# qianlim/CAPE

Hardware: AMD Instinct MI355X
Metric: meshes/sec fwd+bwd, CAPE-affineconv nz64 @ batch 16, 1/2/4/8 MI355X (higher is better)
Workload: dtype f32

## Files before the change

cape_amd/csrc/gconv.hip:

```cpp
#include "common.h"
#include "gconv_shared.h"
#include "gemm_plain.h"
#include "gemm_split.h"
#include "gemm_h2.h"
#include "narrow.h"
#include <stdlib.h>
#include <algorithm>
#include <vector>

namespace {

constexpr int KC_DEFAULT = 32;

template <int ROWS, int LDA, int KC, typename AT = float>
__device__ __forceinline__ void stage_rows(float *sA, const SrcDev &S, int n, int r0, int Mo,
                                            int c0, int tid) {
    constexpr int QPR = KC / 4;
    constexpr int RP = 256 / QPR;
    const int q = tid % QPR;
    const int rl0 = tid / QPR;
    const int c = c0 + 4 * q;
    const AT *x0 = reinterpret_cast<const AT *>(S.x) + (long long)n * S.xs;
    const AT *xb = x0 + c;
    const int nvalid = S.C - c;
// ... 489 lines not shown
    return CAPE_OK;
}

inline int fill_h2(GconvParams &p, const cape_h2_t *h2, bool dual, int out_deinterleave) {
    p.wsi = p.wsi2 = nullptr;
    p.rm_out = nullptr;
    p.rm_out_w = 0;
    if (!h2) return CAPE_OK;
    if (h2->rowmax_out) {
        if (out_deinterleave > 1 || h2->rowmax_out_w < (p.F + 31) / 32 || (h2->rowmax_out_w & 3)) return CAPE_EINVAL;
        p.rm_out = h2->rowmax_out;
        p.rm_out_w = h2->rowmax_out_w;
    }
    if (!h2->src) return CAPE_OK;
    p.wsi = h2->wscale_inv;
    p.wsi2 = dual ? h2->w2scale_inv : nullptr;
    for (int i = 0; i < p.nsrc; ++i) {
        const cape_h2_src_t &h = h2->src[i];
        SrcDev &d = p.s[i];
        d.wh = h.w_hi; d.wl = h.w_lo; d.wp = h.w_pitch;
        d.wh2 = d.w2 ? h.w2_hi : nullptr; d.wl2 = d.w2 ? h.w2_lo : nullptr; d.wp2 = h.w2_pitch;
        d.rm = h.rowmax; d.rmw = h.rowmax_w;
    }
    return CAPE_OK;
}

struct DwPlan {
    int ct, ft, ctiles[CAPE_MAX_SRC], ftiles, ntiles, rsplit, rows_per_split, ngroups, samples_per_group;
    int vstart[CAPE_MAX_SRC + 1];
    long long slab;
};

constexpr int DW_SLOTS_SERIAL = 512, DW_SLOTS_PIPELINED = 256;
inline void plan_dw_splits(int N, int Mo, DwPlan &pl, int slots = DW_SLOTS_SERIAL) {
    int S = slots / pl.ntiles;
    if (S < 1) S = 1;
    int ngroups = 1;
    for (int d = 1; d <= N && d <= S; ++d)
        if (N % d == 0) ngroups = d;
    const int maxr = (Mo + 127) / 128;
    int rsplit = S / ngroups;
    if (rsplit > maxr) rsplit = maxr;
    if (rsplit < 1) rsplit = 1;
    int rows = (Mo + rsplit - 1) / rsplit;
    rows = ((rows + 31) / 32) * 32;
    pl.rows_per_split = rows;
    pl.rsplit = (Mo + rows - 1) / rows;
    pl.samples_per_group = N / ngroups;
    pl.ngroups = ngroups;
}

inline void plan_dw(const cape_src_t *srcs, int nsrc, int N, int Mo, int F, DwPlan &pl) {
    int maxC = 0;
    for (int i = 0; i < nsrc; ++i) maxC = srcs[i].C > maxC ? srcs[i].C : maxC;
    pl.ct = (maxC <= 64) ? 64 : 128;
    pl.ft = (F <= 64) ? 64 : 128;
    pl.ftiles = (F + pl.ft - 1) / pl.ft;
    pl.ntiles = 0;
    pl.slab = 0;
    for (int i = 0; i < nsrc; ++i) {
        pl.ctiles[i] = (srcs[i].C + pl.ct - 1) / pl.ct;
        pl.ntiles += pl.ctiles[i] * pl.ftiles;
        pl.slab += (long long)srcs[i].C * F;
    }
    plan_dw_splits(N, Mo, pl);
}

inline void plan_dw_plain(const cape_src_t *srcs, int nsrc, int N, int Mo, int F, bool pack, DwPlan &pl) {
    int sumC = 0, maxC = 0;
    pl.slab = 0;
    for (int i = 0; i < nsrc; ++i) {
        sumC += srcs[i].C;
        maxC = srcs[i].C > maxC ? srcs[i].C : maxC;
        pl.slab += (long long)srcs[i].C * F;
    }
    const int span = pack ? sumC : maxC;
    const int n128 = (span + 127) / 128, n64 = (span + 63) / 64;
    pl.ft = (F <= 32) ? 32 : (F <= 64) ? 64 : 128;
    pl.ct = (pl.ft == 32 || n64 == 2 * n128) ? 128 : 64;
    pl.ftiles = (F + pl.ft - 1) / pl.ft;
    int v = 0;
    for (int i = 0; i < nsrc; ++i) {
        if (!pack) v = (v + pl.ct - 1) / pl.ct * pl.ct;
        pl.vstart[i] = v;
        v += srcs[i].C;
    }
    pl.vstart[nsrc] = v;
    pl.ntiles = ((v + pl.ct - 1) / pl.ct) * pl.ftiles;
    plan_dw_splits(N, Mo, pl);
}

inline bool dw_srcs_plain(const cape_src_t *srcs, int nsrc, int es = 4) {
    for (int i = 0; i < nsrc; ++i)
        if ((((srcs[i].C + 3) & ~3) > srcs[i].ldx) || (srcs[i].ldx & 3) || (srcs[i].x_sample_stride & 3) ||
            (reinterpret_cast<uintptr_t>(srcs[i].x) & (4 * es - 1)))
            return false;
    return true;
}


inline bool dw_dz_vec(const float *dz, int64_t dz_sample_stride, int32_t lddz, const float *dz2, int es = 4) {
    return ((lddz & 3) == 0) && ((dz_sample_stride & 3) == 0) && ((reinterpret_cast<uintptr_t>(dz) & (4 * es - 1)) == 0) &&
           (!dz2 || (reinterpret_cast<uintptr_t>(dz2) & (4 * es - 1)) == 0);
}

inline void fill_h2_dw(DwParams &p, const cape_h2_dw_t *h2) {
    p.dzrm = p.dz2rm = nullptr;
    p.dzrmw = p.dz2rmw = 0;
    if (!h2) return;
    for (int i = 0; i < p.nsrc; ++i) { p.s[i].rm = h2->src_rowmax[i]; p.s[i].rmw = h2->src_rowmax_w[i]; }
    p.dzrm = h2->dz_rowmax; p.dzrmw = h2->dz_rowmax_w;
    p.dz2rm = h2->dz2_rowmax; p.dz2rmw = h2->dz2_rowmax_w;
}

inline int choose_dw(const cape_src_t *srcs, int nsrc, const float *dz, int64_t dz_sample_stride, int32_t lddz,
                     const float *dz2, uint32_t dz2_mask, int N, int Mo, int F, DwPlan &pl, bool bf16 = false) {
    static const int dwp_on = getenv("CAPE_DW_PLAIN") ? atoi(getenv("CAPE_DW_PLAIN")) : 1;
    const int es = bf16 ? 2 : 4;
    const bool dzvec = dw_dz_vec(dz, dz_sample_stride, lddz, dz2, es);
    const bool plain = dwp_on && dzvec && (((F + 3) & ~3) <= lddz) && dw_srcs_plain(srcs, nsrc, es);
    if (bf16) {
        bool c4b = true;
        int sumCb = 0;
        for (int i = 0; i < nsrc; ++i) { c4b = c4b && (srcs[i].C & 3) == 0; sumCb += srcs[i].C; }
        if (plain && c4b && (F & 1) == 0) {
            plan_dw(srcs, nsrc, N, Mo, F, pl);
            return 3;
        }
        if (plain && c4b && !(dz2 && dz2_mask) && nsrc > 1 && sumCb <= 128 && F <= 64) {
            plan_dw_plain(srcs, nsrc, N, Mo, F, true, pl);
            return 2;
        }
        plan_dw(srcs, nsrc, N, Mo, F, pl);
        return plain ? 1 : 0;
    }
    int sumC = 0;
    for (int i = 0; i < nsrc; ++i) sumC += srcs[i].C;
    bool c4 = true;
    for (int i = 0; i < nsrc; ++i) c4 = c4 && (srcs[i].C & 3) == 0;
    const bool packed = plain && c4 && !(dz2 && dz2_mask) && nsrc > 1 && sumC <= 128 && F <= 64;
    static const int dws_on = getenv("CAPE_DW_BF16X6") ? atoi(getenv("CAPE_DW_BF16X6")) : CAPE_DW_BF16X6_DEFAULT;
    const bool dw_split = dws_on && plain && !packed && c4 && (F & 1) == 0;
    if (packed) plan_dw_plain(srcs, nsrc, N, Mo, F, true, pl);
    else plan_dw(srcs, nsrc, N, Mo, F, pl);
    return packed ? 2 : dw_split ? 3 : plain ? 1 : 0;
}

struct FwdPlan {
    int family;
    int BM, BN;
    int layout;
};

inline FwdPlan plan_fwd(const GconvParams &p, const cape_src_t *srcs, bool dual, bool bf16 = false) {
    FwdPlan pl;
    static const int gp_on = getenv("CAPE_GEMM_PLAIN") ? atoi(getenv("CAPE_GEMM_PLAIN")) : 1;
    pl.layout = gp_on ? gp_weight_layout(p, dual) : -1;
    if (bf16) {
        bool ok = pl.layout >= 0 && p.F >= 64;
        for (int i = 0; i < p.nsrc && ok; ++i) {
            const long long ws = srcs[i].w_cs > srcs[i].w_rs ? srcs[i].w_cs : srcs[i].w_rs;
            ok = (srcs[i].ldx & 7) == 0 && (srcs[i].x_sample_stride & 7) == 0 && (reinterpret_cast<uintptr_t>(srcs[i].x) & 15) == 0 &&
                 (long long)p.Mo * srcs[i].ldx < (1LL << 31) && (long long)p.F * ws < (1LL << 31) &&
                 srcs[i].C % GS_KC == 0 && srcs[i].C >= GS_KC;
        }
        if (ok) {
            pl.family = 2;
            gs_tile(dual, p.N, p.Mo, p.F, pl.BM, pl.BN);
            return pl;
        }
        pl.layout = -1;
    }
    for (int i = 0; i < p.nsrc && pl.layout >= 0; ++i) {
        const long long ws = srcs[i].w_cs > srcs[i].w_rs ? srcs[i].w_cs : srcs[i].w_rs;
        if ((long long)p.Mo * srcs[i].ldx >= (1LL << 31) || (long long)p.F * ws >= (1LL << 31)) pl.layout = -1;
    }
    if (pl.layout >= 0 && h2_eligible(p, dual)) {
        pl.family = 3;
        pl.layout = 1;
        int ktot = 0;
        for (int i = 0; i < p.nsrc; ++i) ktot += p.s[i].C;
        h2_tile(dual, p.N, p.Mo, p.F, ktot, pl.BM, pl.BN);
        return pl;
    }
    if (pl.layout >= 0) {
        static const int gs_on = getenv("CAPE_GEMM_BF16X6") ? atoi(getenv("CAPE_GEMM_BF16X6")) : CAPE_GEMM_BF16X6_DEFAULT;
        if (gs_on && gs_eligible(p, dual)) {
            pl.family = 2;
            gs_tile(dual, p.N, p.Mo, p.F, pl.BM, pl.BN);
            return pl;
        }
        static const int narrow_on = getenv("CAPE_NARROW") ? atoi(getenv("CAPE_NARROW")) : 1;
        int sumC = 0;
        for (int i = 0; i < p.nsrc; ++i) sumC += p.s[i].C;
        if (narrow_on && !dual && sumC <= NARROW_MAXC && (p.F & 3) == 0 && p.F >= 16 && p.F <= 256 &&
            (long long)p.N * p.Mo < (1LL << 31)) {
            pl.family = 4;
            pl.BM = 256 / narrow_lpr(p.F / 4); pl.BN = p.F;
            return pl;
        }
        pl.family = 1;
        gp_tile(dual, p.F, pl.BM, pl.BN);
        return pl;
    }
    pl.family = 0;
    pl.BN = (p.F <= 32) ? 32 : (p.F <= 64 || dual) ? 64 : 128;
    pl.BM = 128;
    constexpr int bm64_below = 640;
    if (pl.BN == 128 && (long long)p.N * ((p.Mo + 127) / 128) * ((p.F + 127) / 128) < bm64_below) pl.BM = 64;
    return pl;
}

inline int fill_fwd_srcs(GconvParams &p, const cape_src_t *srcs, int nsrc, bool &dual, int es = 4) {
    dual = false;
    for (int i = 0; i < nsrc; ++i) {
        if (!srcs[i].w) return CAPE_EINVAL;
        int rc = fill_src(p.s[i], srcs[i], es);
        if (rc) return rc;
        dual = dual || (srcs[i].w2 != nullptr);
    }
    p.nsrc = nsrc;
    return CAPE_OK;
}

}

namespace {

int gconv_fwd_plan_impl(const cape_src_t *srcs, int32_t nsrc, int32_t N, int32_t Mo, int32_t F, int32_t plan[4], bool bf16,
                        const cape_h2_t *h2 = nullptr) {
    if (!srcs || nsrc < 1 || nsrc > CAPE_MAX_SRC || N < 1 || Mo < 1 || F < 1 || !plan) return CAPE_EINVAL;
    GconvParams p;
    bool dual;
    int rc = fill_fwd_srcs(p, srcs, nsrc, dual, bf16 ? 2 : 4);
    if (rc) return rc;
    p.N = N; p.Mo = Mo; p.F = F;
    rc = fill_h2(p, bf16 ? nullptr : h2, dual, 0);
    if (rc) return rc;
    const FwdPlan pl = plan_fwd(p, srcs, dual, bf16);
    plan[0] = pl.family; plan[1] = pl.BM; plan[2] = pl.BN; plan[3] = pl.family ? pl.layout : 0;
    return CAPE_OK;
}

template <typename AT>
void launch_generic_fwd(const GconvParams &p, const FwdPlan &pl, bool dual, dim3 grid, hipStream_t st) {
    const dim3 block(256);
    if (!dual) {
        if (pl.BN == 32) CAPE_LAUNCH((gconv_fwd_kernel<128, 32, 4, 1, false, KC_DEFAULT, AT>), grid, block, 0, st, p);
        else if (pl.BN == 64) CAPE_LAUNCH((gconv_fwd_kernel<128, 64, 4, 1, false, KC_DEFAULT, AT>), grid, block, 0, st, p);
        else if (pl.BM == 64) CAPE_LAUNCH((gconv_fwd_kernel<64, 128, 2, 2, false, KC_DEFAULT, AT>), grid, block, 0, st, p);
        else CAPE_LAUNCH((gconv_fwd_kernel<128, 128, 2, 2, false, KC_DEFAULT, AT>), grid, block, 0, st, p);
    } else {
        if (pl.BN == 32) CAPE_LAUNCH((gconv_fwd_kernel<128, 32, 4, 1, true, KC_DEFAULT, AT>), grid, block, 0, st, p);
        else CAPE_LAUNCH((gconv_fwd_kernel<128, 64, 4, 1, true, KC_DEFAULT, AT>), grid, block, 0, st, p);
    }
}

int gconv_fwd_impl(const cape_src_t *srcs, int32_t nsrc, float *y, int64_t y_sample_stride,
                   int32_t ldy, int32_t N, int32_t Mo, int32_t F, const float *bias,
                   int32_t bias_mode, int32_t act, uint32_t *mask_out, const cape_rank_t *rank,
                   int32_t out_deinterleave, void *stream, bool bf16, const cape_h2_t *h2 = nullptr) {
    if (!srcs || nsrc < 1 || nsrc > CAPE_MAX_SRC || !y || N < 1 || Mo < 1 || F < 1) return CAPE_EINVAL;
    if (bf16 && h2) return CAPE_EINVAL;
    const int dK = out_deinterleave > 1 ? out_deinterleave : 1;
    const int dstride = dK > 1 ? ((F / dK + 3) & ~3) : 0;
    if (dK > 1 && (F % dK != 0 || mask_out || rank || ldy < dK * dstride)) return CAPE_EINVAL;
    if (dK == 1 && ldy < F) return CAPE_EINVAL;
    if (bias_mode != CAPE_BIAS_NONE && !bias) return CAPE_EINVAL;
    if (act < CAPE_ACT_NONE || act > CAPE_ACT_TANH) return CAPE_EINVAL;
    GconvParams p;
    bool dual;
    int rc = fill_fwd_srcs(p, srcs, nsrc, dual, bf16 ? 2 : 4);
    if (rc) return rc;
    if (mask_out && !dual) return CAPE_EINVAL;
    if (dual && (bias_mode != CAPE_BIAS_NONE || act != CAPE_ACT_NONE)) return CAPE_EINVAL;
    p.y = y; p.ys = y_sample_stride; p.ldy = ldy;
    p.N = N; p.Mo = Mo; p.F = F;
    p.bias = bias; p.bias_mode = bias ? bias_mode : CAPE_BIAS_NONE; p.act = act;
    p.mask = mask_out; p.mask_words = (F + 31) / 32;
    p.rankR = 0; p.rowscale = nullptr; p.coef = nullptr; p.rank_to2 = 0;
    p.deintK = dK; p.deint_stride = dstride;
    if (rank && rank->R > 0) {
        if (rank->R > CAPE_MAX_SRC || !rank->rowscale || !rank->coef) return CAPE_EINVAL;
        if (rank->to_acc2 && !dual) return CAPE_EINVAL;
        p.rankR = rank->R; p.rowscale = rank->rowscale; p.coef = rank->coef; p.rank_to2 = rank->to_acc2;
    }
    rc = fill_h2(p, h2, dual, dK);
    if (rc) return rc;
    FwdPlan pl = plan_fwd(p, srcs, dual, bf16);
    if (pl.family == 4) {
        const bool ok = !p.rankR && !p.mask && dK == 1 && !p.rm_out && (ldy & 3) == 0 && (y_sample_stride & 3) == 0 &&
                        (reinterpret_cast<uintptr_t>(y) & 15) == 0 && (!p.bias || (reinterpret_cast<uintptr_t>(p.bias) & 15) == 0);
        if (ok) {
            const int lpr = narrow_lpr(F / 4), RL = 256 / lpr;
            long long blocks = ((long long)N * Mo + 4 * RL - 1) / (4 * RL);
            if (blocks > 1024) blocks = 1024;
            CAPE_LAUNCH(fwd_narrow_in_kernel, dim3((unsigned)blocks), dim3(256), (size_t)NARROW_MAXC * 4 * lpr * sizeof(float),
                        (hipStream_t)stream, p, lpr);
            CAPE_LAUNCH_CHECK();
            return CAPE_OK;
        }
        pl.family = 1;
        gp_tile(dual, p.F, pl.BM, pl.BN);
    }
    p.row_tiles = (Mo + pl.BM - 1) / pl.BM;
    p.col_tiles = (F + pl.BN - 1) / pl.BN;
    dim3 grid((unsigned)(N * p.row_tiles * p.col_tiles));
    hipStream_t st = (hipStream_t)stream;
    if (pl.family == 3) {
        h2_launch(p, dual, pl.BM, pl.BN, grid, st);
    } else if (pl.family == 2) {
        gs_launch(p, dual, pl.BM, pl.layout, bf16, grid, st);
    } else if (pl.family == 1) {
        gp_launch(p, dual, pl.BM, pl.BN, pl.layout, grid, st);
    } else if (bf16) {
        launch_generic_fwd<cape_bf16>(p, pl, dual, grid, st);
    } else {
        launch_generic_fwd<float>(p, pl, dual, grid, st);
    }
    CAPE_LAUNCH_CHECK();
    return CAPE_OK;
}

}

extern "C" int cape_gconv_fwd_plan(const cape_src_t *srcs, int32_t nsrc, int32_t N, int32_t Mo, int32_t F, int32_t plan[4]) {
    return gconv_fwd_plan_impl(srcs, nsrc, N, Mo, F, plan, false);
}

extern "C" int cape_gconv_fwd_plan_bf16(const cape_src_t *srcs, int32_t nsrc, int32_t N, int32_t Mo, int32_t F, int32_t plan[4]) {
    return gconv_fwd_plan_impl(srcs, nsrc, N, Mo, F, plan, true);
}

extern "C" int cape_gconv_fwd(const cape_src_t *srcs, int32_t nsrc, float *y, int64_t y_sample_stride,
                              int32_t ldy, int32_t N, int32_t Mo, int32_t F, const float *bias,
                              int32_t bias_mode, int32_t act, uint32_t *mask_out, const cape_rank_t *rank,
                              int32_t out_deinterleave, void *stream) {
    return gconv_fwd_impl(srcs, nsrc, y, y_sample_stride, ldy, N, Mo, F, bias, bias_mode, act, mask_out, rank, out_deinterleave,
                          stream, false);
}

extern "C" int cape_gconv_fwd_h2(const cape_src_t *srcs, int32_t nsrc, float *y, int64_t y_sample_stride,
                                 int32_t ldy, int32_t N, int32_t Mo, int32_t F, const float *bias,
                                 int32_t bias_mode, int32_t act, uint32_t *mask_out, const cape_rank_t *rank,
                                 int32_t out_deinterleave, const cape_h2_t *h2, void *stream) {
    return gconv_fwd_impl(srcs, nsrc, y, y_sample_stride, ldy, N, Mo, F, bias, bias_mode, act, mask_out, rank, out_deinterleave,
                          stream, false, h2);
}

extern "C" int cape_gconv_fwd_plan_h2(const cape_src_t *srcs, int32_t nsrc, int32_t N, int32_t Mo, int32_t F, const cape_h2_t *h2,
                                      int32_t plan[4]) {
    return gconv_fwd_plan_impl(srcs, nsrc, N, Mo, F, plan, false, h2);
}

extern "C" int cape_gconv_fwd_bf16(const cape_src_t *srcs, int32_t nsrc, void *y, int64_t y_sample_stride,
                                   int32_t ldy, int32_t N, int32_t Mo, int32_t F, const float *bias,
                                   int32_t bias_mode, int32_t act, uint32_t *mask_out, const cape_rank_t *rank,
                                   int32_t out_deinterleave, void *stream) {
    return gconv_fwd_impl(srcs, nsrc, (float *)y, y_sample_stride, ldy, N, Mo, F, bias, bias_mode, act, mask_out, rank,
                          out_deinterleave, stream, true);
}

extern "C" int64_t cape_gconv_dw_workspace_bytes(const cape_src_t *srcs, int32_t nsrc, int32_t N,
                                                 int32_t Mo, int32_t F) {
    if (!srcs || nsrc < 1 || nsrc > CAPE_MAX_SRC || N < 1 || Mo < 1 || F < 1) return CAPE_EINVAL;
    DwPlan pl;
    plan_dw(srcs, nsrc, N, Mo, F, pl);
    long long need = pl.slab * pl.ngroups * pl.rsplit;
    {
        plan_dw_plain(srcs, nsrc, N, Mo, F, true, pl);
        const long long n2 = pl.slab * pl.ngroups * pl.rsplit;
        need = n2 > need ? n2 : need;
    }
    return (int64_t)need * (int64_t)sizeof(float);
}

namespace {
inline bool dw_takes_h2(const cape_src_t *srcs, int nsrc, const float *dz2, uint32_t dz2_mask, int Mo, int lddz, const cape_h2_dw_t *h2) {
    if (!h2) return false;
    DwParams p;
    p.nsrc = nsrc;
    p.dz2_mask = dz2 ? dz2_mask : 0u;
    p.Mo = Mo; p.lddz = lddz;
    for (int i = 0; i < nsrc; ++i) p.s[i].ldx = srcs[i].ldx;
    fill_h2_dw(p, h2);
    return h2_dw_eligible(p);
}
int gconv_dw_plan_impl(const cape_src_t *srcs, int32_t nsrc, const float *dz, int64_t dz_sample_stride,
                       int32_t lddz, const float *dz2, uint32_t dz2_mask, int32_t N, int32_t Mo, int32_t F,
                       int32_t plan[4], bool bf16, const cape_h2_dw_t *h2 = nullptr) {
    if (!srcs || nsrc < 1 || nsrc > CAPE_MAX_SRC || !dz || N < 1 || Mo < 1 || F < 1 || lddz < F || !plan) return CAPE_EINVAL;
    DwPlan pl;
    plan[0] = choose_dw(srcs, nsrc, dz, dz_sample_stride, lddz, dz2, dz2_mask, N, Mo, F, pl, bf16);
    const int nm = dw_narrow_mode(srcs, nsrc, dz, dz_sample_stride, lddz, dz2, dz2_mask, F, plan[0], bf16);
    if (nm) {
        plan[0] = nm;
    } else if (plan[0] == 3 && !bf16 && dw_takes_h2(srcs, nsrc, dz2, dz2_mask, Mo, lddz, h2)) {
        plan[0] = 4;
        plan_dw_splits(N, Mo, pl, DW_SLOTS_PIPELINED);
    }
    plan[1] = pl.ct; plan[2] = pl.ft; plan[3] = pl.ngroups * pl.rsplit;
    return CAPE_OK;
}
struct DwReduceParams;
struct DwDescribe {
    DwParams p;
    DwPlan pl;
    bool use_h2, v4;
};
int gconv_dw_stage_impl(const cape_src_t *srcs, int32_t nsrc, const float *dz,
                        int64_t dz_sample_stride, int32_t lddz, const float *dz2, uint32_t dz2_mask,
                        int32_t N, int32_t Mo, int32_t F, int32_t accumulate, void *workspace,
                        int64_t workspace_bytes, int32_t stage, void *stream, bool bf16,
                        DwReduceParams *batch_rp = nullptr, int *batch_vec = nullptr, int *batch_blocks = nullptr,
                        const cape_h2_dw_t *h2 = nullptr, DwDescribe *describe = nullptr);
}

extern "C" int cape_gconv_dw_plan(const cape_src_t *srcs, int32_t nsrc, const float *dz, int64_t dz_sample_stride,
                                  int32_t lddz, const float *dz2, uint32_t dz2_mask, int32_t N, int32_t Mo, int32_t F,
                                  int32_t plan[4]) {
    return gconv_dw_plan_impl(srcs, nsrc, dz, dz_sample_stride, lddz, dz2, dz2_mask, N, Mo, F, plan, false);
}

extern "C" int cape_gconv_dw_plan_h2(const cape_src_t *srcs, int32_t nsrc, const float *dz, int64_t dz_sample_stride,
                                     int32_t lddz, const float *dz2, uint32_t dz2_mask, int32_t N, int32_t Mo, int32_t F,
                                     const cape_h2_dw_t *h2, int32_t plan[4]) {
    return gconv_dw_plan_impl(srcs, nsrc, dz, dz_sample_stride, lddz, dz2, dz2_mask, N, Mo, F, plan, false, h2);
}

extern "C" int cape_gconv_dw_stage_h2(const cape_src_t *srcs, int32_t nsrc, const float *dz,
                                      int64_t dz_sample_stride, int32_t lddz, const float *dz2, uint32_t dz2_mask,
                                      int32_t N, int32_t Mo, int32_t F, int32_t accumulate, void *workspace,
                                      int64_t workspace_bytes, int32_t stage, const cape_h2_dw_t *h2, void *stream) {
    if (stage > 2) return CAPE_EINVAL;
    return gconv_dw_stage_impl(srcs, nsrc, dz, dz_sample_stride, lddz, dz2, dz2_mask, N, Mo, F, accumulate, workspace,
                               workspace_bytes, stage, stream, false, nullptr, nullptr, nullptr, h2);
}

extern "C" int cape_gconv_dw_plan_bf16(const cape_src_t *srcs, int32_t nsrc, const void *dz, int64_t dz_sample_stride,
                                       int32_t lddz, const void *dz2, uint32_t dz2_mask, int32_t N, int32_t Mo, int32_t F,
                                       int32_t plan[4]) {
    return gconv_dw_plan_impl(srcs, nsrc, (const float *)dz, dz_sample_stride, lddz, (const float *)dz2, dz2_mask, N, Mo, F, plan, true);
}

extern "C" int cape_gconv_dw_bf16(const cape_src_t *srcs, int32_t nsrc, const void *dz,
                                  int64_t dz_sample_stride, int32_t lddz, const void *dz2, uint32_t dz2_mask,
                                  int32_t N, int32_t Mo, int32_t F, int32_t accumulate, void *workspace,
                                  int64_t workspace_bytes, void *stream) {
    return gconv_dw_stage_impl(srcs, nsrc, (const float *)dz, dz_sample_stride, lddz, (const float *)dz2, dz2_mask, N, Mo, F,
                               accumulate, workspace, workspace_bytes, 0, stream, true);
}

extern "C" int cape_gconv_dw_stage_bf16(const cape_src_t *srcs, int32_t nsrc, const void *dz,
                                        int64_t dz_sample_stride, int32_t lddz, const void *dz2, uint32_t dz2_mask,
                                        int32_t N, int32_t Mo, int32_t F, int32_t accumulate, void *workspace,
                                        int64_t workspace_bytes, int32_t stage, void *stream) {
// ... 339 lines not shown
```

cape_amd/csrc/narrow.h:

```cpp
#pragma once

constexpr int NARROW_MAXC = 8;

struct NarrowTab {
    const float *xp[NARROW_MAXC];
    long long xss[NARROW_MAXC];
    int xld[NARROW_MAXC];
};
template <typename P>
__device__ __forceinline__ void narrow_table(const P &p, NarrowTab &t) {
#pragma unroll
    for (int j = 0; j < NARROW_MAXC; ++j) {
        int jj = j, si = 0;
        while (si < p.nsrc && jj >= p.s[si].C) { jj -= p.s[si].C; ++si; }
        const bool on = si < p.nsrc;
        t.xp[j] = on ? p.s[si].x + jj : p.s[0].x;
        t.xss[j] = on ? p.s[si].xs : p.s[0].xs;
        t.xld[j] = on ? p.s[si].ldx : p.s[0].ldx;
    }
}

__global__ __launch_bounds__(256) void fwd_narrow_in_kernel(GconvParams p, int lpr) {
    extern __shared__ float wl[];
    const int FS = 4 * lpr;
    for (int o = threadIdx.x; o < NARROW_MAXC * FS; o += 256) wl[o] = 0.f;
    __syncthreads();
    int sc = 0;
    for (int si = 0; si < p.nsrc; ++si) {
        const SrcDev &S = p.s[si];
        for (int o = threadIdx.x; o < S.C * FS; o += 256) {
            const int c = o / FS, f = o % FS;
            if (f < p.F) wl[(sc + c) * FS + f] = S.w[(long long)c * S.wrs + (long long)f * S.wcs];
        }
        sc += S.C;
    }
    __syncthreads();
    NarrowTab T;
    narrow_table(p, T);
    const int fq = threadIdx.x % lpr, rl = threadIdx.x / lpr, RL = 256 / lpr;
    const int f = 4 * fq;
    const unsigned rows = (unsigned)p.N * (unsigned)p.Mo;
    float4 wq[NARROW_MAXC];
#pragma unroll
    for (int j = 0; j < NARROW_MAXC; ++j) wq[j] = *reinterpret_cast<const float4 *>(&wl[j * FS + f]);
    float4 bq = make_float4(0.f, 0.f, 0.f, 0.f);
    if (p.bias_mode == CAPE_BIAS_CHANNEL && f < p.F) bq = *reinterpret_cast<const float4 *>(p.bias + f);
    constexpr int UR = 4;
    for (unsigned nr0 = blockIdx.x * RL * UR + rl; nr0 < rows; nr0 += gridDim.x * RL * UR) {
        float xv[UR][NARROW_MAXC];
        unsigned nq[UR], rq[UR];
#pragma unroll
        for (int u = 0; u < UR; ++u) {
            const unsigned nr = min(nr0 + u * RL, rows - 1);
            nq[u] = nr / (unsigned)p.Mo;
            rq[u] = nr - nq[u] * (unsigned)p.Mo;
#pragma unroll
            for (int j = 0; j < NARROW_MAXC; ++j) xv[u][j] = T.xp[j][(long long)nq[u] * T.xss[j] + (long long)rq[u] * T.xld[j]];
        }
        __builtin_amdgcn_sched_barrier(0);
#pragma unroll
        for (int u = 0; u < UR; ++u) {
            float4 a = bq;
            if (p.bias_mode == CAPE_BIAS_VERTEX && f < p.F) a = *reinterpret_cast<const float4 *>(p.bias + (long long)rq[u] * p.F + f);
#pragma unroll
            for (int j = 0; j < NARROW_MAXC; ++j) {
                a.x = fmaf(xv[u][j], wq[j].x, a.x); a.y = fmaf(xv[u][j], wq[j].y, a.y);
                a.z = fmaf(xv[u][j], wq[j].z, a.z); a.w = fmaf(xv[u][j], wq[j].w, a.w);
            }
            a.x = cape_act(a.x, p.act); a.y = cape_act(a.y, p.act); a.z = cape_act(a.z, p.act); a.w = cape_act(a.w, p.act);
            if (f < p.F && nr0 + u * RL < rows)
                *reinterpret_cast<float4 *>(p.y + (long long)nq[u] * p.ys + (long long)rq[u] * p.ldy + f) = a;
        }
    }
}

__global__ __launch_bounds__(256) void dw_narrow_in_kernel(DwParams p, int lpr, int ntiles) {
    extern __shared__ float red[];
    int tile, split;
    if (!cape_map_dw_block(blockIdx.x, ntiles, p.ngroups * p.rsplit, tile, split) || tile != 0) return;
    const int grp = split / p.rsplit, rs = split % p.rsplit;
    const int n_begin = grp * p.samples_per_group, n_end = min(p.N, n_begin + p.samples_per_group);
    const int ra = rs * p.rows_per_split, rb = min(p.Mo, ra + p.rows_per_split);
    const int FS = 4 * lpr, RL = 256 / lpr;
    const int fq = threadIdx.x % lpr, rl = threadIdx.x / lpr;
    const int f = 4 * fq;
    const bool fon = f < p.F;
    NarrowTab T;
    narrow_table(p, T);
    float acc[NARROW_MAXC][4];
#pragma unroll
    for (int j = 0; j < NARROW_MAXC; ++j) acc[j][0] = acc[j][1] = acc[j][2] = acc[j][3] = 0.f;
    constexpr int UR = 4;
    for (int n = n_begin; n < n_end; ++n) {
        const float *zb = p.dz + (long long)n * p.dzs + (fon ? f : 0);
        for (int r0 = ra + rl; r0 < rb; r0 += UR * RL) {
            float4 d[UR];
            float xv[UR][NARROW_MAXC];
#pragma unroll
            for (int u = 0; u < UR; ++u) {
                const int rc = min(r0 + u * RL, rb - 1);
                d[u] = *reinterpret_cast<const float4 *>(zb + (long long)rc * p.lddz);
#pragma unroll
                for (int j = 0; j < NARROW_MAXC; ++j) xv[u][j] = T.xp[j][(long long)n * T.xss[j] + (long long)rc * T.xld[j]];
            }
            __builtin_amdgcn_sched_barrier(0);
#pragma unroll
            for (int u = 0; u < UR; ++u) {
                const float okf = (r0 + u * RL < rb && fon) ? 1.f : 0.f;
                const float4 dd = make_float4(d[u].x * okf, d[u].y * okf, d[u].z * okf, d[u].w * okf);
#pragma unroll
                for (int j = 0; j < NARROW_MAXC; ++j) {
                    acc[j][0] = fmaf(xv[u][j], dd.x, acc[j][0]); acc[j][1] = fmaf(xv[u][j], dd.y, acc[j][1]);
                    acc[j][2] = fmaf(xv[u][j], dd.z, acc[j][2]); acc[j][3] = fmaf(xv[u][j], dd.w, acc[j][3]);
                }
            }
        }
    }
#pragma unroll
    for (int j = 0; j < NARROW_MAXC; ++j)
        *reinterpret_cast<float4 *>(&red[(rl * NARROW_MAXC + j) * FS + f]) = make_float4(acc[j][0], acc[j][1], acc[j][2], acc[j][3]);
    __syncthreads();
    float *out = p.ws + (long long)split * p.slab;
    int j0 = 0;
    for (int si = 0; si < p.nsrc; ++si) {
        const int Cs = p.s[si].C;
        for (int o = threadIdx.x; o < Cs * lpr; o += 256) {
            const int c = o / lpr, q = o % lpr;
            if (4 * q >= p.F) continue;
            float4 s = make_float4(0.f, 0.f, 0.f, 0.f);
            for (int l = 0; l < RL; ++l) {
                const float4 v = *reinterpret_cast<const float4 *>(&red[(l * NARROW_MAXC + j0 + c) * FS + 4 * q]);
                s.x += v.x; s.y += v.y; s.z += v.z; s.w += v.w;
            }
            *reinterpret_cast<float4 *>(out + p.part_off[si] + (long long)c * p.F + 4 * q) = s;
        }
        j0 += Cs;
    }
}

__global__ __launch_bounds__(256) void dw_narrow_out_kernel(DwParams p, int lpr, int ntiles) {
    extern __shared__ float red[];
    int tile, split;
    if (!cape_map_dw_block(blockIdx.x, ntiles, p.ngroups * p.rsplit, tile, split) || tile != 0) return;
    const int grp = split / p.rsplit, rs = split % p.rsplit;
    const int n_begin = grp * p.samples_per_group, n_end = min(p.N, n_begin + p.samples_per_group);
    const int ra = rs * p.rows_per_split, rb = min(p.Mo, ra + p.rows_per_split);
    const int RL = 256 / lpr;
    const int cq = threadIdx.x % lpr, rl = threadIdx.x / lpr;
    int si = 0, c0 = 4 * cq;
    while (si < p.nsrc && c0 >= p.s[si].C) { c0 -= p.s[si].C; ++si; }
    const bool con = si < p.nsrc;
    const SrcDev &S = p.s[con ? si : 0];
    float acc[4][4];
#pragma unroll
    for (int i = 0; i < 4; ++i) acc[i][0] = acc[i][1] = acc[i][2] = acc[i][3] = 0.f;
    for (int n = n_begin; n < n_end; ++n) {
        const float *zb = p.dz + (long long)n * p.dzs;
        const float *xb = S.x + (long long)n * S.xs + (con ? c0 : 0);
        constexpr int UR = 4;
        for (int r0 = ra + rl; r0 < rb; r0 += UR * RL) {
            float d[UR][4];
            float4 xq[UR];
#pragma unroll
            for (int u = 0; u < UR; ++u) {
                const int r = r0 + u * RL;
                const float okf = (r < rb && con) ? 1.f : 0.f;
                const int rc = min(r, rb - 1);
#pragma unroll
                for (int f = 0; f < 4; ++f) d[u][f] = zb[(long long)rc * p.lddz + min(f, p.F - 1)] * (f < p.F ? okf : 0.f);
                xq[u] = *reinterpret_cast<const float4 *>(xb + (long long)rc * S.ldx);
            }
#pragma unroll
            for (int u = 0; u < UR; ++u) {
                const float xa[4] = {xq[u].x, xq[u].y, xq[u].z, xq[u].w};
#pragma unroll
                for (int i = 0; i < 4; ++i)
#pragma unroll
                    for (int f = 0; f < 4; ++f) acc[i][f] = fmaf(xa[i], d[u][f], acc[i][f]);
            }
        }
    }
#pragma unroll
    for (int i = 0; i < 4; ++i)
        *reinterpret_cast<float4 *>(&red[((rl * lpr + cq) * 4 + i) * 4]) = make_float4(acc[i][0], acc[i][1], acc[i][2], acc[i][3]);
    __syncthreads();
    if (rl == 0 && con) {
        float *out = p.ws + (long long)split * p.slab + p.part_off[si];
#pragma unroll
        for (int i = 0; i < 4; ++i) {
            float4 s = make_float4(0.f, 0.f, 0.f, 0.f);
            for (int l = 0; l < RL; ++l) {
                const float4 v = *reinterpret_cast<const float4 *>(&red[((l * lpr + cq) * 4 + i) * 4]);
                s.x += v.x; s.y += v.y; s.z += v.z; s.w += v.w;
            }
            const float sv[4] = {s.x, s.y, s.z, s.w};
            for (int f = 0; f < p.F; ++f) out[(long long)(c0 + i) * p.F + f] = sv[f];
        }
    }
}

inline int narrow_lpr(int quads) {
    int l = 1;
    while (l < quads) l <<= 1;
    return l;
}

inline int dw_narrow_mode(const cape_src_t *srcs, int nsrc, const float *dz, int64_t dz_sample_stride, int32_t lddz, const float *dz2,
                          uint32_t dz2_mask, int F, int fam, bool bf16) {
    static const int on = getenv("CAPE_NARROW") ? atoi(getenv("CAPE_NARROW")) : 1;
    if (!on || bf16 || fam == 0 || (dz2 && dz2_mask)) return 0;
    int sumC = 0;
    bool c4 = true, xal = true;
    for (int i = 0; i < nsrc; ++i) {
        sumC += srcs[i].C;
        c4 = c4 && (srcs[i].C & 3) == 0;
        xal = xal && (srcs[i].ldx & 3) == 0 && (srcs[i].x_sample_stride & 3) == 0 && (reinterpret_cast<uintptr_t>(srcs[i].x) & 15) == 0;
    }
    const bool dzal = (lddz & 3) == 0 && (dz_sample_stride & 3) == 0 && (reinterpret_cast<uintptr_t>(dz) & 15) == 0;
    if (sumC <= NARROW_MAXC && (F & 3) == 0 && F >= 16 && F <= 256 && dzal) return 5;
    if (F <= 4 && c4 && xal && sumC >= 16 && sumC <= 256) return 6;
    return 0;
}
```

cape_amd/ops.py:

```python
import ctypes as C

import numpy as np
import torch

from . import _lib
from ._lib import lib, CapeSrc, check
from .graph import ConvOperators, HostCSR

import os as _os
FUSED_RECURRENCE = int(_os.environ.get("CAPE_FUSED_RECURRENCE", "1"))
CMR_FUSED_TAIL = int(_os.environ.get("CAPE_CMR_FUSED_TAIL", "1"))
MERGED_D_PASS = _os.environ.get("CAPE_MERGED_D_PASS", "auto")


def merged_d_pass(batch):
    if MERGED_D_PASS == "auto":
        return 2 * int(batch) <= 32
    return bool(int(MERGED_D_PASS))
SPMM_ELL = int(_os.environ.get("CAPE_SPMM_ELL", "1"))

_ACT_OF = {"b1leakyrelu": ("leaky", _lib.BIAS_CHANNEL), "b1relu": ("relu", _lib.BIAS_CHANNEL),
           "b1tanh": ("tanh", _lib.BIAS_CHANNEL), "b2relu": ("relu", _lib.BIAS_VERTEX)}


# ... 87 lines not shown
        self.nnz = host.nnz
        self.max_row, self.min_row = host.max_row, host.min_row
        if not host.identity:
            rc = lib.cape_csr_validate(host.shape[0], host.shape[1], host.nnz,
                                       host.rowptr.ctypes.data_as(C.c_void_p),
                                       host.colidx.ctypes.data_as(C.c_void_p))
            check(rc, "cape_csr_validate")
        self.rowptr_t = torch.from_numpy(host.rowptr).to(device)
        self.colidx_t = torch.from_numpy(host.colidx if host.nnz else np.zeros(1, np.int32)).to(device)
        self.vals_t = torch.from_numpy(host.vals if host.nnz else np.zeros(1, np.float32)).to(device)
        self.ell_w, self.ell_col_t, self.ell_val_t = 0, None, None
        ell = ell_arrays(host)
        if ell is not None:
            self.ell_w = int(ell[0].shape[1])
            self.ell_col_t = torch.from_numpy(ell[0]).to(device)
            self.ell_val_t = torch.from_numpy(ell[1]).to(device)

    def operands(self):
        if SPMM_ELL and self.ell_w:
            return self.rowptr_t.data_ptr(), self.ell_col_t.data_ptr(), self.ell_val_t.data_ptr(), self.ell_w
        return self.rowptr_t.data_ptr(), self.colidx_t.data_ptr(), self.vals_t.data_ptr(), 0


class DeviceConvOps(object):

    def __init__(self, host, device):
        assert isinstance(host, ConvOperators)
        self.K, self.fused = host.K, host.fused
        self.Mi, self.Mo = host.Mi, host.Mo
        if host.fused:
            self.fwd = [DeviceCSR(h, device) for h in host.fwd]
            self.bwd = [DeviceCSR(h, device) for h in host.bwd]
            rs = host.cond_row_terms()
            self.rowscale = torch.from_numpy(np.stack(rs + [rs[0]]).astype(np.float32)).to(device).contiguous()
        else:
            self.Lt = DeviceCSR(host.Lt, device)
            self.LtT = DeviceCSR(host.LtT, device)
        self.host = host
        self.device = device
        self._patch_plans = {}

    def patch_plan(self, Cin, Fout):
        key = (int(Cin), int(Fout))
        if key not in self._patch_plans:
            plan = None
            host = self.host
            ok = (not self.fused and host.unfused_unpool is None and host.unfused_pool is None
                  and lib.cape_cheb_fused_supported(int(Cin), int(Fout), int(self.K)) == 1)
            if ok:
                from .graph import ChebPatchPlan
                Lt = host.Lt.to_scipy()
                if abs(Lt - Lt.T).max() <= 1e-6 * max(abs(Lt).max(), 1e-30):
                    try:
                        plan = DevicePatchPlan(ChebPatchPlan(Lt, self.K, Cin, reserve_bytes=8 * 4 * int(Cin) * int(Fout)), self.device)
                    except ValueError:
                        plan = None
            self._patch_plans[key] = plan
        return self._patch_plans[key]


class DevicePatchPlan(object):
    def __init__(self, host, device):
        self.host = host
        self.P, self.rmax, self.K, self.M = host.P, host.rmax, host.K, host.M
        t = lambda a: torch.from_numpy(np.ascontiguousarray(a)).to(device)
        self.pinfo, self.vid, self.ell_col, self.ell_val = t(host.pinfo), t(host.vid), t(host.ell_col), t(host.ell_val)


def _mk_srcs(entries):
    arr = (CapeSrc * len(entries))()
    for s, e in zip(arr, entries):
        x = e["x"]
        p, ss, ld = _v(x)
        s.x, s.x_sample_stride, s.ldx, s.C = p, ss, ld, int(e.get("C", x.shape[2]))
        wt, off, rs, cs = e["w"]
        s.w, s.w_rs, s.w_cs = wt.data_ptr() + 4 * int(off), int(rs), int(cs)
        if e.get("w2") is not None:
            wt2, off2, rs2, cs2 = e["w2"]
            s.w2, s.w2_rs, s.w2_cs = wt2.data_ptr() + 4 * int(off2), int(rs2), int(cs2)
        else:
            s.w2, s.w2_rs, s.w2_cs = None, 0, 0
    return arr


LAUNCH_LOG = None
PLAN_LOG = None
ACT_TRACE = None
L1_SIGN_TRACE = None


def _trace_sign(y, act):
    if ACT_TRACE is not None and act in ("leaky", "relu"):
        ACT_TRACE.append((y.detach() > 0).cpu())


def _trace_mask_bits(mask, F):
    if ACT_TRACE is not None:
        sh = torch.arange(32, device=mask.device, dtype=torch.int32)
        bits = ((mask.unsqueeze(-1) >> sh) & 1).reshape(mask.shape[0], mask.shape[1], -1)[:, :, :F]
        ACT_TRACE.append((bits != 0).cpu())


def _gconv_work(entries, N, Mo, F):
    es = entries[0]["x"].element_size()
    flops, byts = 0, es * N * Mo * F
    seen = set()
    for e in entries:
        Cs = int(e.get("C", e["x"].shape[2]))
        nblk = 2 if e.get("w2") is not None else 1
        flops += 2 * N * Mo * Cs * F * nblk
        byts += 4 * Cs * F * nblk
        key = e["x"].data_ptr()
        if key not in seen:
            seen.add(key)
            byts += es * N * e["x"].shape[1] * Cs
    return flops, byts


def _dw_work(entries, N, Mo, F, two_dz):
    es = entries[0]["x"].element_size()
    flops, byts = 0, es * N * Mo * F * (2 if two_dz else 1)
    seen = set()
    for e in entries:
        Cs = int(e.get("C", e["x"].shape[2]))
        flops += 2 * N * Mo * Cs * F
        byts += 4 * Cs * F
        key = e["x"].data_ptr()
        if key not in seen:
            seen.add(key)
            byts += es * N * e["x"].shape[1] * Cs
    return flops, byts


def _csr_bytes(csr):
    return 0 if (csr is None or csr.identity) else 8 * csr.nnz + 4 * (csr.shape[0] + 1)


LOG_SPACER_US = int(_os.environ.get("CAPE_LOG_SPACER_US", "80"))


def _log_launch(name, flops, byts, fn):
    if LAUNCH_LOG is None:
        return fn()
    e0, e1 = torch.cuda.Event(enable_timing=True), torch.cuda.Event(enable_timing=True)
    if LOG_SPACER_US:
        lib.cape_spin_us(LOG_SPACER_US, _stream())
    e0.record()
    out = fn()
    e1.record()
    LAUNCH_LOG.append((name, int(flops), int(byts), e0, e1))
    return out


_FWD_FAMILY = {0: "gconv_fwd_kernel", 1: "gemm_plain_kernel", 2: "gemm_split_kernel", 3: "gemm_h2_kernel", 4: "fwd_narrow_in_kernel"}
_DW_FAMILY = {0: "gconv_dw_kernel", 1: "dw_plain_kernel", 2: "dw_packed_kernel", 3: "dw_split_kernel", 4: "dw_h2_kernel",
              5: "dw_narrow_in_kernel", 6: "dw_narrow_out_kernel"}


def fwd_kernel_name(fam, bm, bn, layout, dual, bf16=False):
    waves = "2, 2" if (bm, bn) in ((64, 128), (128, 128), (64, 64)) else "4, 1"
    tf = lambda b: "true" if b else "false"
    at = ", unsigned short" if bf16 else ", float"
    if fam == 4:
        return "fwd_narrow_in_kernel"
    if fam == 3:
        if (bm, bn) == (128, 256) and not dual:
            return "gemm_h2x_kernel<0, 0>"
        return "gemm_h2_kernel<%d, %d, %s>" % (bm, bn, tf(dual))
    if fam == 2:
        return "gemm_split_kernel<%d, %d, %s, %s%s>" % (bm, bn, tf(layout), tf(dual), at)
    if fam == 1:
        return "gemm_plain_kernel<%d, %d, %s, %s, %s>" % (bm, bn, waves, tf(dual), tf(layout))
    return "gconv_fwd_kernel<%d, %d, %s, %s, 32%s>" % (bm, bn, waves, tf(dual), at)


def dw_kernel_name(fam, ct, ft, bf16=False):
    if fam in (5, 6):
        return _DW_FAMILY[fam]
    if fam == 4:
        return "dw_h2_kernel<%d, %d, %s>" % (ct, ft, "true" if (DW_V4 and (ct, ft) == (128, 128)) else "false")
    if fam == 3 or fam == 0:
        return "%s<%d, %d, %s>" % (_DW_FAMILY[fam], ct, ft, "unsigned short" if bf16 else "float")
    waves = "4, 1" if (fam == 2 and ft == 32) else "2, 2"
    return "%s<%d, %d, %s, %s>" % (_DW_FAMILY[fam], ct, ft, waves, "unsigned short" if bf16 else "float")


FUSE_ACT_GRAD = int(_os.environ.get("CAPE_FUSE_ACT_GRAD", "1"))
FUSE_PREP_SPMM = int(_os.environ.get("CAPE_FUSE_PREP_SPMM", "1"))
DW_V4 = int(_os.environ.get("CAPE_DW_V4", "1"))
DW_BATCH = int(_os.environ.get("CAPE_DW_BATCH", "1"))
_CHAIN = [False]


class _ActOffer(object):
    __slots__ = ("act", "gB", "fused")

    def __init__(self, act, gB):
        self.act, self.gB, self.fused = act, gB, False


class sole_consumer_chain(object):
    def __init__(self, on=True):
        self.on = bool(on)

    def __enter__(self):
        self.prev, _CHAIN[0] = _CHAIN[0], self.on
        return self

    def __exit__(self, *exc):
        _CHAIN[0] = self.prev
        return False


H2 = int(_os.environ.get("CAPE_H2", "1"))
RM_TRACE = int(_os.environ.get("CAPE_RM_TRACE", "0"))


def rm_width(F):
    return ((int(F) + 31) // 32 + 3) // 4 * 4


def alloc_rm(t, F=None):
    return torch.empty((t.shape[0], t.shape[1], rm_width(t.shape[2] if F is None else F)), device=t.device, dtype=torch.float32)


def set_rm(t, rm):
    if rm is not None:
        t._cape_rm = rm
        t._cape_rm_version = t._version
    return t


def drop_rm(t):
    if getattr(t, "_cape_rm", None) is not None:
        t._cape_rm = None


def rm_of(t):
    rm = getattr(t, "_cape_rm", None)
    if rm is None or rm.shape[0] != t.shape[0] or rm.shape[1] != t.shape[1] or rm.device != t.device:
        return None
    if getattr(t, "_cape_rm_version", None) != t._version:
        return None
    return rm


def h2_shape_ok(ktot, F):
    return F >= 64 and (ktot >= 256 or (ktot >= 128 and F >= 128))


def _want_rm(t, Cn=None, any_width=False):
    Cn = t.shape[2] if Cn is None else Cn
    if not (bool(H2) and t.dtype == torch.float32 and Cn % 32 == 0 and Cn >= 32):
        return False
    return any_width or (Cn & (Cn - 1)) == 0


def _new_rm(t):
    return torch.empty((t.shape[0], t.shape[1], 4), device=t.device, dtype=torch.float32)


def rowmax(t):
    rm = rm_of(t)
    if rm is not None:
        return rm
    _lib.require_gpu()
    t = as_act(t)
    assert t.dtype == torch.float32
    if RM_TRACE:
        import traceback
        print("standalone rowmax for", tuple(t.shape), "<-", " <- ".join("%s:%d" % (f.name, f.lineno) for f in traceback.extract_stack()[-6:-1]), flush=True)
    rm = torch.empty((t.shape[0], t.shape[1], 4), device=t.device, dtype=torch.float32)
    p, ss, ld = _v(t)
    _log_launch("rowmax_kernel", 0, 4 * t.shape[0] * t.shape[1] * (t.shape[2] + 4),
                lambda: check(lib.cape_rowmax(p, ss, ld, t.shape[0], t.shape[1], t.shape[2], _ptr(rm), 4, _stream()), "cape_rowmax"))
    set_rm(t, rm)
    return rm


class WeightPieces(object):
    __slots__ = ("W", "Ch", "K", "F", "pair", "fpair", "f_hi", "f_lo", "b_hi", "b_lo", "fsi", "bsi", "bsc")

    def fwd(self, k):
        o = 2 * k * self.F * self.Ch
        return self.f_hi.data_ptr() + o, self.f_lo.data_ptr() + o, self.Ch

    def bwd(self, k):
        o = 2 * k * self.F
        return self.b_hi.data_ptr() + o, self.b_lo.data_ptr() + o, self.K * self.F


class PiecePlan(object):

    def __init__(self, specs, device):
        self.items, sizes = [], []
        for sp in specs:
            W, Ch, K = sp["W"], int(sp["Ch"]), int(sp["K"])
            F = int(W.shape[1])
            assert W.is_contiguous() and W.dtype == torch.float32 and W.shape[0] >= Ch * K and Ch % 8 == 0 and F % 8 == 0
            sizes.append((Ch, K, F))
        al = lambda nbytes: (nbytes + 255) // 256 * 256
        rpatch = lambda sp, Ch, K: (Ch * K + (int(sp["fpair"][1]) if sp.get("fpair") is not None else 0) + 63) // 64
        total = sum(4 * al(2 * Ch * K * F) + al(4 * K * F) + al(4 * Ch * K) + al(4 * Ch) + al(4 * rpatch(sp, Ch, K) * F)
                    for sp, (Ch, K, F) in zip(specs, sizes))
        self.arena = torch.empty(max(total, 256), device=device, dtype=torch.uint8)
        off = 0

        def take(nbytes, dtype):
            nonlocal off
            t = self.arena[off:off + nbytes].view(dtype)
            off += al(nbytes)
            return t

        arr = (_lib.CapeWpieceItem * len(specs))()
        for a, sp, (Ch, K, F) in zip(arr, specs, sizes):
            wp = WeightPieces()
            wp.W, wp.Ch, wp.K, wp.F, wp.pair, wp.fpair = sp["W"], Ch, K, F, sp.get("pair"), sp.get("fpair")
# ... 1990 lines not shown
```

Before: 6307.

## Add narrow-output forward kernel for tiny-F gconv and extend narrow-in routing

Adds fwd_narrow_out_kernel for forward graph convolutions with at most 4 output channels and 32-128 input channels. Lanes split the input channels, each does a 4x4 FMA block, and partial sums are reduced across lanes with DPP. Bias and low-rank terms are folded into that same reduction, and the kernel uses a persistent grid with software-prefetched loads. The planner also sends narrow-input cases to the narrow-in kernel when plain GEMM is off but the weights are transposed, and falls back by re-planning instead of forcing the plain GEMM. The aim is to avoid wasting GEMM tiles on outputs only a few columns wide (e.g. final xyz layers), at the cost of extra kernel-selection complexity.

Measured after the change: 6337, median of 6. No clear change (+0.5%).

```diff
diff --git a/cape_amd/csrc/gconv.hip b/cape_amd/csrc/gconv.hip
--- a/cape_amd/csrc/gconv.hip
+++ b/cape_amd/csrc/gconv.hip
@@ -665,10 +665,30 @@
     int layout;
 };
 
-inline FwdPlan plan_fwd(const GconvParams &p, const cape_src_t *srcs, bool dual, bool bf16 = false) {
+inline FwdPlan plan_fwd(const GconvParams &p, const cape_src_t *srcs, bool dual, bool bf16 = false, bool narrow = true) {
     FwdPlan pl;
     static const int gp_on = getenv("CAPE_GEMM_PLAIN") ? atoi(getenv("CAPE_GEMM_PLAIN")) : 1;
     pl.layout = gp_on ? gp_weight_layout(p, dual) : -1;
+    static const int narrow_env = getenv("CAPE_NARROW") ? atoi(getenv("CAPE_NARROW")) : 1;
+    const bool narrow_on = narrow && narrow_env && !dual && !bf16;
+    int sumC = 0;
+    bool c4 = true, xvec = true, wT = true;
+    for (int i = 0; i < p.nsrc; ++i) {
+        sumC += p.s[i].C;
+        c4 = c4 && (p.s[i].C & 3) == 0;
+        xvec = xvec && p.s[i].vec;
+        wT = wT && p.s[i].wrs == 1;
+    }
+    if (narrow_on && p.F <= 4 && c4 && xvec && sumC >= 32 && sumC <= 128) {
+        const int RL = 256 / narrow_lpr(sumC / 4);
+        if ((long long)p.N * ((p.Mo + 4 * RL - 1) / (4 * RL)) < (1LL << 31)) {
+            pl.family = 5;
+            pl.BM = 4 * RL; pl.BN = 4;
+            return pl;
+        }
+    }
+    const bool narrow_in = narrow_on && sumC <= NARROW_MAXC && (p.F & 3) == 0 && p.F >= 16 && p.F <= 256 &&
+                           (long long)p.N * p.Mo < (1LL << 31);
     if (bf16) {
         bool ok = pl.layout >= 0 && p.F >= 64;
         for (int i = 0; i < p.nsrc && ok; ++i) {
@@ -703,17 +723,18 @@
             gs_tile(dual, p.N, p.Mo, p.F, pl.BM, pl.BN);
             return pl;
         }
-        static const int narrow_on = getenv("CAPE_NARROW") ? atoi(getenv("CAPE_NARROW")) : 1;
-        int sumC = 0;
-        for (int i = 0; i < p.nsrc; ++i) sumC += p.s[i].C;
-        if (narrow_on && !dual && sumC <= NARROW_MAXC && (p.F & 3) == 0 && p.F >= 16 && p.F <= 256 &&
-            (long long)p.N * p.Mo < (1LL << 31)) {
+        if (narrow_in) {
             pl.family = 4;
             pl.BM = 256 / narrow_lpr(p.F / 4); pl.BN = p.F;
             return pl;
         }
         pl.family = 1;
         gp_tile(dual, p.F, pl.BM, pl.BN);
+        return pl;
+    }
+    if (narrow_in && wT) {
+        pl.family = 4;
+        pl.BM = 256 / narrow_lpr(p.F / 4); pl.BN = p.F;
         return pl;
     }
     pl.family = 0;
@@ -813,8 +834,21 @@
             CAPE_LAUNCH_CHECK();
             return CAPE_OK;
         }
-        pl.family = 1;
-        gp_tile(dual, p.F, pl.BM, pl.BN);
+        pl = plan_fwd(p, srcs, dual, bf16, false);
+    } else if (pl.family == 5) {
+        const bool ok = !p.mask && dK == 1 && !p.rm_out && p.rankR <= NARROW_MAXR;
+        if (ok) {
+            int sumC = 0;
+            for (int i = 0; i < nsrc; ++i) sumC += srcs[i].C;
+            const int lpr = narrow_lpr(sumC / 4), RL = 256 / lpr;
+            const int chunks = (Mo + 4 * RL - 1) / (4 * RL);
+            const long long tiles = (long long)N * chunks, per = (tiles + 1023) / 1024;
+            const long long blocks = (tiles + per - 1) / per;
+            CAPE_LAUNCH(fwd_narrow_out_kernel, dim3((unsigned)blocks), dim3(256), 0, (hipStream_t)stream, p, lpr, chunks);
+            CAPE_LAUNCH_CHECK();
+            return CAPE_OK;
+        }
+        pl = plan_fwd(p, srcs, dual, bf16, false);
     }
     p.row_tiles = (Mo + pl.BM - 1) / pl.BM;
     p.col_tiles = (F + pl.BN - 1) / pl.BN;
diff --git a/cape_amd/csrc/narrow.h b/cape_amd/csrc/narrow.h
--- a/cape_amd/csrc/narrow.h
+++ b/cape_amd/csrc/narrow.h
@@ -71,6 +71,102 @@
             if (f < p.F && nr0 + u * RL < rows)
                 *reinterpret_cast<float4 *>(p.y + (long long)nq[u] * p.ys + (long long)rq[u] * p.ldy + f) = a;
         }
+    }
+}
+
+constexpr int NARROW_MAXR = 4;
+
+__device__ __forceinline__ float narrow_row_sum(float v, int lpr) {
+#define CAPE_DPP_ADD(v, CTRL) ((v) + __builtin_bit_cast(float, __builtin_amdgcn_update_dpp(0, __builtin_bit_cast(int, (v)), (CTRL), 0xF, 0xF, false)))
+    v = CAPE_DPP_ADD(v, 0xB1);
+    v = CAPE_DPP_ADD(v, 0x4E);
+    v = CAPE_DPP_ADD(v, 0x141);
+    if (lpr >= 16) v = CAPE_DPP_ADD(v, 0x140);
+    if (lpr >= 32) v = cape_sum_xor16(v);
+#undef CAPE_DPP_ADD
+    return v;
+}
+
+__global__ __launch_bounds__(256) void fwd_narrow_out_kernel(GconvParams p, int lpr, int chunks) {
+    const int RL = 256 / lpr;
+    const int cq = threadIdx.x % lpr, rl = threadIdx.x / lpr;
+    const float *sx = p.s[0].x, *sw = p.s[0].w;
+    long long sxs = p.s[0].xs, swrs = p.s[0].wrs, swcs = p.s[0].wcs;
+    int sldx = p.s[0].ldx, c0 = 0, base = 0;
+    bool con = false;
+#pragma unroll
+    for (int i = 0; i < CAPE_MAX_SRC; ++i) {
+        if (i >= p.nsrc) break;
+        const SrcDev &Si = p.s[i];
+        const bool m = 4 * cq >= base && 4 * cq < base + Si.C;
+        sx = m ? Si.x : sx; sw = m ? Si.w : sw;
+        sxs = m ? Si.xs : sxs; swrs = m ? Si.wrs : swrs; swcs = m ? Si.wcs : swcs;
+        sldx = m ? Si.ldx : sldx; c0 = m ? 4 * cq - base : c0;
+        con = con || m;
+        base += Si.C;
+    }
+    float w[4][4];
+#pragma unroll
+    for (int i = 0; i < 4; ++i)
+#pragma unroll
+        for (int f = 0; f < 4; ++f) w[i][f] = sw[(long long)(c0 + i) * swrs + (long long)min(f, p.F - 1) * swcs];
+    const bool is_b = p.bias_mode != CAPE_BIAS_NONE && cq < p.F;
+    const bool is_r = cq >= 4 && cq - 4 < p.rankR;
+    const float *ep = is_b ? p.bias + cq : is_r ? p.rowscale + (long long)(cq - 4) * p.Mo : sx;
+    const int es = is_b ? (p.bias_mode == CAPE_BIAS_VERTEX ? p.F : 0) : is_r ? 1 : 0;
+    const float *cp = is_r ? p.coef + (long long)(cq - 4) * p.F : sw;
+    const long long cs = is_r ? (long long)p.rankR * p.F : 0;
+    const int cf = is_r ? 1 : 0;
+    constexpr int UR = 4;
+    const int tiles = p.N * chunks;
+    auto loads = [&](int t, float4 (&xq)[UR], float (&e)[UR], float (&ew)[4]) {
+        const int n = t / chunks, r0 = (t - n * chunks) * (RL * UR) + rl;
+        const float *xb = sx + (long long)n * sxs + c0;
+#pragma unroll
+        for (int f = 0; f < 4; ++f) ew[f] = cp[(long long)n * cs + min(f, p.F - 1) * cf];
+#pragma unroll
+        for (int u = 0; u < UR; ++u) {
+            const int rc = min(r0 + u * RL, p.Mo - 1);
+            xq[u] = *reinterpret_cast<const float4 *>(xb + (long long)rc * sldx);
+            e[u] = ep[(long long)rc * es];
+        }
+    };
+    float4 xq[UR], xn[UR];
+    float e[UR], en[UR], ew[4], ewn[4];
+    if ((int)blockIdx.x < tiles) loads(blockIdx.x, xq, e, ew);
+    __builtin_amdgcn_sched_barrier(0);
+#pragma unroll
+    for (int i = 0; i < 4; ++i)
+#pragma unroll
+        for (int f = 0; f < 4; ++f) w[i][f] = (con && f < p.F) ? w[i][f] : 0.f;
+    for (int t = blockIdx.x; t < tiles; t += gridDim.x) {
+        const int n = t / chunks, r0 = (t - n * chunks) * (RL * UR) + rl;
+        if (t + (int)gridDim.x < tiles) loads(t + gridDim.x, xn, en, ewn);
+        __builtin_amdgcn_sched_barrier(0);
+#pragma unroll
+        for (int f = 0; f < 4; ++f) ew[f] = is_r ? ew[f] : (is_b && f == cq) ? 1.f : 0.f;
+#pragma unroll
+        for (int u = 0; u < UR; ++u) {
+            const int r = r0 + u * RL;
+            const float ev = (is_b || is_r) ? e[u] : 0.f;
+            float a[4];
+#pragma unroll
+            for (int f = 0; f < 4; ++f) {
+                float s = xq[u].x * w[0][f];
+                s = fmaf(xq[u].y, w[1][f], s); s = fmaf(xq[u].z, w[2][f], s); s = fmaf(xq[u].w, w[3][f], s);
+                a[f] = f < p.F ? narrow_row_sum(fmaf(ev, ew[f], s), lpr) : 0.f;
+            }
+            if (cq == 0 && r < p.Mo) {
+                float *yr = p.y + (long long)n * p.ys + (long long)r * p.ldy;
+#pragma unroll
+                for (int f = 0; f < 4; ++f)
+                    if (f < p.F) yr[f] = p.act == CAPE_ACT_NONE ? a[f] : cape_act(a[f], p.act);
+            }
+        }
+#pragma unroll
+        for (int u = 0; u < UR; ++u) { xq[u] = xn[u]; e[u] = en[u]; }
+#pragma unroll
+        for (int f = 0; f < 4; ++f) ew[f] = ewn[f];
     }
 }
 
diff --git a/cape_amd/ops.py b/cape_amd/ops.py
--- a/cape_amd/ops.py
+++ b/cape_amd/ops.py
@@ -263,7 +263,8 @@
     return out
 
 
-_FWD_FAMILY = {0: "gconv_fwd_kernel", 1: "gemm_plain_kernel", 2: "gemm_split_kernel", 3: "gemm_h2_kernel", 4: "fwd_narrow_in_kernel"}
+_FWD_FAMILY = {0: "gconv_fwd_kernel", 1: "gemm_plain_kernel", 2: "gemm_split_kernel", 3: "gemm_h2_kernel", 4: "fwd_narrow_in_kernel",
+               5: "fwd_narrow_out_kernel"}
 _DW_FAMILY = {0: "gconv_dw_kernel", 1: "dw_plain_kernel", 2: "dw_packed_kernel", 3: "dw_split_kernel", 4: "dw_h2_kernel",
               5: "dw_narrow_in_kernel", 6: "dw_narrow_out_kernel"}
 
@@ -272,8 +273,8 @@
     waves = "2, 2" if (bm, bn) in ((64, 128), (128, 128), (64, 64)) else "4, 1"
     tf = lambda b: "true" if b else "false"
     at = ", unsigned short" if bf16 else ", float"
-    if fam == 4:
-        return "fwd_narrow_in_kernel"
+    if fam in (4, 5):
+        return _FWD_FAMILY[fam]
     if fam == 3:
         if (bm, bn) == (128, 256) and not dual:
             return "gemm_h2x_kernel<0, 0>"
```
